# linjonathan/tropical_cyclone_risk

Measured on AMD Instinct MI355X. Metric: storm-steps/sec (100k-storm ensemble), higher is better.
Workload: dtype f64

## Files before the change

### tropical_cyclone_risk_amd/csrc/tcr_abi.hip

```cpp
#include <hip/hip_runtime.h>

#include <atomic>
#include <chrono>
#include <cmath>
#include <condition_variable>
#include <memory>
#include <mutex>
#include <thread>
#include <cstdio>
#include <cstdlib>
#include <cstring>
#include <string>
#include <vector>

#include "tcr_kernels.hip"
#include "tcr_seed.hip"
#include "tcr_compact.hip"
#include "tcr_prep.hip"
#include "tcr_thermo.hip"
#ifdef TCR_EXPERIMENTS
#include "tcr_experiments.h"
#endif

using namespace tcr;
// ... 611 lines not shown
    const bool f64 = std::is_same<R, double>::value;
    if (ctx->split_static) { K.bx = axis_of<R>(ctx->bg, true); K.by = axis_of<R>(ctx->bg, false); }
    else { K.bx = K.hx; K.by = K.hy; }
    switch (ctx->static_mode) {
    case kStatF64Split:
        K.stat = f64 ? static_cast<const void *>(ctx->d_land) : static_cast<const void *>(ctx->d_land32);
        K.bathy = f64 ? static_cast<const void *>(ctx->d_bathy) : static_cast<const void *>(ctx->d_bathy32);
        break;
    case kStatPack16: case kStatPack64: K.stat = ctx->d_nstat; K.bathy = nullptr; break;
    case kStatU8F32: K.stat = ctx->d_nstat; K.bathy = ctx->d_nbathy; break;
    default:
        K.stat = f64 ? static_cast<const void *>(ctx->d_stat) : static_cast<const void *>(ctx->d_stat32);
        K.bathy = nullptr;
        break;
    }
    eval_k_scalars<R>(ctx->prm, K);
    K.tw_same = (ctx->wg.lon == ctx->tg.lon && ctx->wg.lat == ctx->tg.lat) ? 1 : 0;
    K.hb_same = ctx->split_static ? 0 : 1;
    *all_affine = K.wx.affine && K.wy.affine && K.tx.affine && K.ty.affine && K.hx.affine && K.hy.affine &&
                  K.bx.affine && K.by.affine;
}

int widen_static(tcr_ctx *ctx, hipStream_t st)
{
    const int mode = ctx->static_mode;
    if (mode != kStatPack16 && mode != kStatU8F32 && mode != kStatPack64) return 0;
    if (ctx->capturing) return fail(ctx, "internal: static fields would be widened inside a stream capture");
    const size_t np = ctx->hg.lon.size() * ctx->hg.lat.size();
    const size_t nb = ctx->split_static ? ctx->bg.lon.size() * ctx->bg.lat.size() : np;
    if (ctx->split_static) { if (dev_alloc(ctx, &ctx->d_land, np) || dev_alloc(ctx, &ctx->d_bathy, nb)) return -1; }
    else if (dev_alloc(ctx, &ctx->d_stat, np * kStaticStride)) return -1;
    hipLaunchKernelGGL(k_static_widen, dim3((unsigned)((std::max(np, nb) + 255) / 256)), dim3(256), 0, st, mode, ctx->d_nstat, ctx->d_nbathy,
                       np, nb, ctx->d_stat, ctx->d_land, ctx->d_bathy);
    HIPCHK(ctx, hipGetLastError());
    HIPCHK(ctx, hipStreamSynchronize(st));
    HIPCHK(ctx, hipFree(ctx->d_nstat)); ctx->d_nstat = nullptr;
    if (ctx->d_nbathy) { HIPCHK(ctx, hipFree(ctx->d_nbathy)); ctx->d_nbathy = nullptr; }
    ctx->static_mode = ctx->split_static ? kStatF64Split : kStatF64;
    ctx->static_bytes = sizeof(double) * (np + nb);
    ctx->stat32_stale = true;
    ++ctx->epoch;
    return 0;
}

template <typename R>
int eval_k_ready(tcr_ctx *ctx, EvalKT<R> &K, bool *affine, hipStream_t st)
{
    host_eval_k<R>(ctx, K, affine);
    if (!*affine && (ctx->static_mode == kStatPack16 || ctx->static_mode == kStatU8F32 || ctx->static_mode == kStatPack64)) {
        if (widen_static(ctx, st)) return -1;
        if (!std::is_same<R, double>::value && ensure_f32(ctx, st)) return -1;
        host_eval_k<R>(ctx, K, affine);
    }
    return 0;
}

template <typename R>
struct TracksT {
    R *lon, *lat, *v, *m, *vmax, *envw;
    int32_t *n_valid, *status, *flags, *nfev, *n_accept, *n_reject, *pad_state;
    int32_t tc_rows_only;
};
template <typename R, typename T>
TracksT<R> tracks_of(const T *o)
{
    TracksT<R> t{};
    t.lon = o->lon; t.lat = o->lat; t.v = o->v; t.m = o->m; t.vmax = o->vmax; t.envw = o->envw;
    t.n_valid = o->n_valid; t.status = o->status; t.flags = o->flags; t.nfev = o->nfev;
    t.n_accept = o->n_accept; t.n_reject = o->n_reject; t.pad_state = o->pad_state; t.tc_rows_only = o->tc_rows_only;
    return t;
}

constexpr int kFsSegSamples = kFsMfmaWaves * kFsMfmaColTiles * 16;
enum FsPart { kFsAll = -1, kFsFirst = 0, kFsRest = 1 };
bool fourier_on_matrix_cores(const tcr_ctx *ctx)
{
    const tcr_params &P = ctx->prm;
    return TCR_FS_MFMA && ctx->fs_period > 0 && 2 * P.n_series <= 4 * kFsMfmaKSteps && P.n_steps <= kFsMfmaMaxSamples;
}

template <typename R>
int launch_fourier(tcr_ctx *ctx, int64_t n, const int64_t *n_dev, const double *phases, R *fs, hipStream_t st,
                   FsPart part = kFsAll, const double *park = nullptr, const unsigned long long *park_count = nullptr,
                   const BatchReset *reset = nullptr)
{
    BatchReset z{};
    if (reset) z = *reset;
    if (reset && !(ctx->fs_period > 0 && fourier_on_matrix_cores(ctx)))
        hipLaunchKernelGGL(k_batch_reset, dim3((unsigned)((std::max<int64_t>(z.n_flags, z.queue_words) + 255) / 256)), dim3(256), 0, st, z);
    const tcr_params &P = ctx->prm;
    if (ctx->fs_period > 0) {
        const size_t lds = sizeof(double2) * (size_t)ctx->fs_period;
        const int64_t nf = n * 4 * (int64_t)P.n_series;
        if (part != kFsRest) {
            double *p = reinterpret_cast<double *>(ctx->d_pf);
            if (grow(ctx, &p, &ctx->pf_cap, (size_t)nf * 2)) { ctx->d_pf = nullptr; return -1; }
            ctx->d_pf = reinterpret_cast<double2 *>(p);
        } else if (!ctx->d_pf) return fail(ctx, "internal: second table segment without the first");
        if (fourier_on_matrix_cores(ctx)) {
            const int64_t tiles = (n + 3) / 4;
            const int64_t *list = nullptr;
            int list_stride = 1;
            if (part == kFsRest) {
                list = reinterpret_cast<const int64_t *>(park) + 13;
                list_stride = kParkRec;
            } else {
                double *p0 = reinterpret_cast<double *>(ctx->d_pf);
                if (grow(ctx, &p0, &ctx->pf_cap, (size_t)tiles * kFsMfmaKSteps * 64)) { ctx->d_pf = nullptr; return -1; }
                ctx->d_pf = reinterpret_cast<double2 *>(p0);
                hipLaunchKernelGGL(k_phase_factors_frag, dim3((unsigned)std::min<int64_t>(tiles, 8192)), dim3(256), 0, st, P, n, n_dev, phases, p0, nullptr, nullptr, z);
            }
            double *p = reinterpret_cast<double *>(ctx->d_pf);
            const int groups = part == kFsAll ? kFsMfmaColGroups : 1;
            int64_t want = (int64_t)ctx->cu_count * kFsMfmaWgsPerCu * (4 / kFsMfmaWaves) / groups;
#ifdef TCR_EXPERIMENTS
            want = tcr_exp::fs_workgroups(want, groups);
#endif
            const unsigned wgs = (unsigned)std::min<int64_t>(tiles, std::max<int64_t>(1, want));
            if (part == kFsRest)
                hipLaunchKernelGGL((k_fourier_mfma<R, true>), dim3(wgs, groups), dim3(64 * kFsMfmaWaves), 0, st, P, n, n_dev, ctx->fs_period,
                                   ctx->d_sc_table, p, fs, 1, list, list_stride, park_count);
            else
                hipLaunchKernelGGL((k_fourier_mfma<R, false>), dim3(wgs, groups), dim3(64 * kFsMfmaWaves), 0, st, P, n, n_dev, ctx->fs_period,
                                   ctx->d_sc_table, p, fs, 0, list, list_stride, park_count);
        } else {
            hipLaunchKernelGGL(k_phase_factors, dim3((unsigned)((nf + 255) / 256)), dim3(256), 0, st, P, n, n_dev, phases, ctx->d_pf);
            hipLaunchKernelGGL(k_fourier_periodic<R>, dim3((unsigned)n), dim3(kFsThreads), lds, st, P, n, n_dev,
                               ctx->fs_period, ctx->d_sc_table, ctx->d_pf, fs);
        }
    } else {
        const int64_t total = n * (int64_t)P.n_steps;
        hipLaunchKernelGGL(k_fourier_direct<R>, dim3((unsigned)((total + 255) / 256)), dim3(256), 0, st, P, n, n_dev, phases, fs);
    }
    HIPCHK(ctx, hipGetLastError());
    return 0;
}

template <typename R>
int integrate_impl(tcr_ctx *ctx, const tcr_storms *in, const TracksT<R> out, void *stream_, uint64_t *stats = nullptr,
                   const int64_t *stats_n_dev = nullptr, int64_t n_expected = 0)
{
    HIPCHK(ctx, hipSetDevice(ctx->device));
    const int64_t n = in->n;
    if (n < 0) return fail(ctx, "tcr_integrate: negative n");
    if (n == 0) return 0;
    hipStream_t st = stream_ ? (hipStream_t)stream_ : ctx->stream;
    const tcr_params &P = ctx->prm;
    const size_t ns = (size_t)P.n_steps;
    constexpr size_t REC = (size_t)step_rec_doubles<R>();
    if (grow(ctx, &ctx->d_fs, &ctx->fs_cap, ((size_t)n * ns * 4 * sizeof(R) + 7) / 8)) return -1;
    const int max_rk = P.max_rk_steps > 0 ? P.max_rk_steps : 64;
    if (grow(ctx, &ctx->d_srec, &ctx->srec_cap, (size_t)n * max_rk * REC)) return -1;
    if (grow(ctx, &ctx->d_vrec, &ctx->vrec_cap, (size_t)n * max_rk * kVRec)) return -1;
    if (max_rk > 65535) return fail(ctx, "tcr_params.max_rk_steps must be <= 65535");
    {
        double *p = reinterpret_cast<double *>(ctx->d_sidx);
        if (grow(ctx, &p, &ctx->sidx_cap, ((size_t)n * ns * sizeof(uint16_t) + 7) / 8)) { ctx->d_sidx = nullptr; return -1; }
        ctx->d_sidx = reinterpret_cast<uint16_t *>(p);
    }
    R *fs = reinterpret_cast<R *>(ctx->d_fs);
    EvalKT<R> EK{};
    bool affine = false;
    if (eval_k_ready<R>(ctx, EK, &affine, st)) return -1;

    hipEvent_t *ev = nullptr;
    if (ctx->timing && !ctx->capturing && timing_events(ctx, &ev)) return -1;
    if (ev) HIPCHK(ctx, hipEventRecord(ev[0], st));
    const int wps = std::is_same<R, double>::value ? TCR_INT_WPS : TCR_INT_WPS_F32;
    unsigned waves = integrate_waves(ctx, (n_expected > 0 && n_expected < n) ? n_expected : n, wps);
    const int thr = park_threshold(ctx, waves, wps);
    const unsigned final_waves = park_final_waves(ctx);
    const bool segmented = kFsMfmaColGroups == 2 && thr > 0 && waves > final_waves && kMaxPasses > 1 && fourier_on_matrix_cores(ctx) &&
                           (int)P.n_steps > kFsSegSamples + 16 && ctx->tune.table_segments != 0;
    int prune_sample = -1;
    if (out.tc_rows_only && ctx->tune.prune != 0) {
        const double t2d = 2 * 86400.0, step_out = P.total_time / (double)(P.n_steps - 1);
        const int j = (int)floor(t2d / step_out);
        if (j >= 1 && j < P.n_steps - 1 && ts_host(P, j) == t2d) {
            prune_sample = j;
            double *q = reinterpret_cast<double *>(ctx->d_screen_skip);
            if (grow(ctx, &q, &ctx->screen_skip_cap, ((size_t)n + 7) / 8)) { ctx->d_screen_skip = nullptr; return -1; }
            ctx->d_screen_skip = reinterpret_cast<uint8_t *>(q);
            double *u = reinterpret_cast<double *>(ctx->d_und_list);
            if (grow(ctx, &u, &ctx->und_list_cap, ((size_t)n + 1) / 2 + 1)) { ctx->d_und_list = nullptr; return -1; }
            ctx->d_und_list = reinterpret_cast<int32_t *>(u);
            if (!ctx->d_und_count && dev_alloc(ctx, &ctx->d_und_count, (size_t)1)) return -1;
        }
    }
    {
        BatchReset z{};
        z.queue = ctx->d_queue; z.queue_words = (int)kQueueWords;
        if (prune_sample >= 0) { z.und_count = ctx->d_und_count; z.flags = out.flags; z.n_flags = n; }
        if (out.tc_rows_only) z.tc_count = reinterpret_cast<unsigned long long *>(ctx->d_tc_count);
        if (launch_fourier<R>(ctx, n, in->n_dev, in->phases, fs, st, segmented ? kFsFirst : kFsAll, nullptr, nullptr, &z)) return -1;
    }
    STAGE(TCR_STAGE_FOURIER);
    if (ev) HIPCHK(ctx, hipEventRecord(ev[1], st));
    {
        KArgsT<R> a{};
        a.P = P; a.D = dev_fields(ctx); a.K = EK; a.n = n; a.n_dev = in->n_dev;
        a.lon0 = in->lon0; a.lat0 = in->lat0; a.v0 = in->v0; a.m0 = in->m0; a.h_bl = in->h_bl;
        a.slot = in->slot; a.phases = in->phases; a.fs = fs; a.srec = ctx->d_srec; a.vrec = ctx->d_vrec; a.max_rk_steps = max_rk;
        a.n_valid = out.n_valid; a.status = out.status; a.nfev = out.nfev;
        a.n_accept = out.n_accept; a.n_reject = out.n_reject;
        a.queue = ctx->d_queue;
        a.prune_sample = prune_sample;
        a.screen_skip = prune_sample >= 0 ? ctx->d_screen_skip : nullptr;
        if (prune_sample >= 0) {
            a.und_list = ctx->d_und_list; a.und_count = ctx->d_und_count;
        }
        const size_t park_items = segmented ? (size_t)n : (size_t)waves * kWave;
        if (thr > 0 && grow(ctx, &ctx->d_park[0], &ctx->park_cap[0], park_items * kParkRec)) return -1;
        if (thr > 0 && grow(ctx, &ctx->d_park[1], &ctx->park_cap[1], park_items * kParkRec)) return -1;
        const bool probe = std::is_same<R, double>::value && ctx->d_probe;
        if (probe) { a.probe = ctx->d_probe; a.probe_cap = ctx->probe_cap; }
        bool seg_events = false;
        for (int pass = 0; pass < kMaxPasses; ++pass) {
            const bool last = thr <= 0 || waves <= final_waves || pass == kMaxPasses - 1;
            a.pass = pass;
            a.fill_pct = pass_fill_pct();
            a.threshold = last ? 0 : thr;
            a.park_in = ctx->d_park[(pass + 1) & 1];
            a.park_out = ctx->d_park[pass & 1];
            a.t_limit = (segmented && pass == 0) ? ts_host(P, kFsSegSamples - 2) : 1e300;
            launch_integrate(a, affine, probe, ctx->static_mode, waves, st);
            if (last) break;
            if (segmented && pass == 0) {
                if (ev) HIPCHK(ctx, hipEventRecord(ev[4], st));
                if (launch_fourier<R>(ctx, n, in->n_dev, in->phases, fs, st, kFsRest, ctx->d_park[0], ctx->d_queue + kMaxPasses)) return -1;
                if (ev) HIPCHK(ctx, hipEventRecord(ev[5], st));
                seg_events = true;
                continue;
            }
            waves = (unsigned)(((size_t)waves * (size_t)(thr - 1) + kWave - 1) / kWave);
        }
        if (ev && !seg_events) { HIPCHK(ctx, hipEventRecord(ev[4], st)); HIPCHK(ctx, hipEventRecord(ev[5], st)); }
    }
    STAGE(TCR_STAGE_INTEGRATE);
    if (ev) HIPCHK(ctx, hipEventRecord(ev[2], st));
    {
        EArgsT<R> a{};
        a.P = P; a.D = dev_fields(ctx); a.n = n; a.n_dev = in->n_dev; a.max_rk_steps = max_rk; a.srec = ctx->d_srec; a.vrec = ctx->d_vrec; a.fs = fs;
        a.slot = in->slot; a.n_valid = out.n_valid; a.status = out.status; a.n_accept = out.n_accept;
        a.lon = out.lon; a.lat = out.lat; a.v = out.v; a.m = out.m; a.vmax = out.vmax;
        a.envw = out.envw; a.flags = out.flags; a.pad_state = out.pad_state;
        a.K = EK;
        a.screen_skip = prune_sample >= 0 ? ctx->d_screen_skip : nullptr;
        if (prune_sample >= 0) { a.und_list = ctx->d_und_list; a.und_count = ctx->d_und_count; }
        const unsigned chunks = (unsigned)((ns + kPostThreads - 1) / kPostThreads);
        if (out.tc_rows_only) {
            if ((size_t)n > ctx->tc_idx_cap) {
                if (ctx->d_tc_idx) HIPCHK(ctx, hipFree(ctx->d_tc_idx));
                ctx->d_tc_idx = nullptr; ctx->tc_idx_cap = 0;
                if (dev_alloc(ctx, &ctx->d_tc_idx, (size_t)n)) return -1;
                ctx->tc_idx_cap = (size_t)n;
            }
            a.tc_list = ctx->d_tc_idx; a.tc_count = reinterpret_cast<unsigned long long *>(ctx->d_tc_count);
            hipLaunchKernelGGL(k_screen<R>, dim3((unsigned)((n + kScreenStorms - 1) / kScreenStorms)), dim3(kScreenThreads), 0, st, a);
            STAGE(TCR_STAGE_SCREEN);
            STAGE(TCR_STAGE_SELECT_TC);
            a.list = ctx->d_tc_idx; a.count = ctx->d_tc_count;
        }
        int64_t cap = kEmitGridCap;
        if (ctx->tune.emit_grid_cap > 0) cap = ctx->tune.emit_grid_cap;
        const unsigned gx = (out.tc_rows_only && n > 2 * cap) ? (unsigned)cap : (unsigned)n;
        hipLaunchKernelGGL(k_dense<R>, dim3(gx), dim3(kWave), 0, st, a, ctx->d_sidx);
        STAGE(TCR_STAGE_DENSE);
        const unsigned ex = gx;
        if (out.tc_rows_only) {
            if (affine) hipLaunchKernelGGL((k_emit<R, true, false>), dim3(ex, chunks), dim3(kPostThreads), 0, st, a, ctx->d_sidx);
            else hipLaunchKernelGGL((k_emit<R, false, false>), dim3(ex, chunks), dim3(kPostThreads), 0, st, a, ctx->d_sidx);
            if ((int64_t)ex < n) {
                a.item_base = ex;
                const unsigned ov = (unsigned)std::min<int64_t>(n - ex, 256);
                if (affine) hipLaunchKernelGGL((k_emit<R, true, true>), dim3(ov, chunks), dim3(kPostThreads), 0, st, a, ctx->d_sidx);
                else hipLaunchKernelGGL((k_emit<R, false, true>), dim3(ov, chunks), dim3(kPostThreads), 0, st, a, ctx->d_sidx);
                a.item_base = 0;
// ... 868 lines not shown
        if (ctx->d_tiles) HIPCHK(ctx, hipFree(ctx->d_tiles));
        ctx->d_tiles = nullptr; ctx->tiles_cap = 0;
        if (dev_alloc(ctx, &ctx->d_tiles, (size_t)tiles + 1024)) return -1;
        HIPCHK(ctx, hipMemsetAsync(ctx->d_tiles, 0, sizeof(unsigned long long) * ((size_t)tiles + 1024), st));
        ctx->tiles_cap = (size_t)tiles + 1024;
    }
    if (cell) hipLaunchKernelGGL(k_compact<true>, dim3((unsigned)tiles), dim3(kScanThreads), 0, st, n, flags, mask, max_out, idx, count, ctx->d_tiles, (int)tiles, *cell);
    else hipLaunchKernelGGL(k_compact<false>, dim3((unsigned)tiles), dim3(kScanThreads), 0, st, n, flags, mask, max_out, idx, count, ctx->d_tiles, (int)tiles, CellOrderArgs{});
    HIPCHK(ctx, hipGetLastError());
    return 0;
}
}
}

int tcr_compact_dev(tcr_ctx *ctx, int64_t n, const int32_t *flags, int32_t mask, int64_t max_out,
                    int32_t *idx, int64_t *count, void *stream_)
{
    return compact_impl(ctx, n, flags, mask, max_out, idx, count, stream_, nullptr);
}

extern "C++" {
namespace {
int cell_order_args(tcr_ctx *ctx, const tcr_seeds *cand, int32_t *idx, int64_t n, const int64_t *count, double cell_deg,
                    hipStream_t st, CellOrderArgs &a)
{
    if (!cand || !cand->lon0 || !cand->lat0 || !idx || n < 0) return fail(ctx, "tcr_cell_order_dev: bad argument");
    if (!(cell_deg >= 0.25 && cell_deg <= 90.0)) return fail(ctx, "tcr_cell_order_dev: cell_deg must be in [0.25, 90]");
    a = CellOrderArgs{};
    a.ncol = (int)ceil(360.0 / cell_deg);
    const int nrow = (int)ceil(180.0 / cell_deg) + 1;
    a.nbins = a.ncol * nrow;
    if (a.nbins > (1 << 20)) return fail(ctx, "tcr_cell_order_dev: too many cells");
    const size_t head = 3 * ((size_t)a.nbins + 1) + 8;
    const size_t words = head + 4 * (size_t)n;
    if ((words + 1) / 2 > ctx->cell_cap || ctx->cell_bins != a.nbins) {
        if (grow(ctx, &ctx->d_cell, &ctx->cell_cap, (words + 1) / 2 + 4096)) return -1;
        HIPCHK(ctx, hipMemsetAsync(ctx->d_cell, 0, sizeof(int32_t) * head, st));
        ctx->cell_bins = a.nbins;
        ctx->cell_counts_open = false;
    } else if (ctx->cell_counts_open && !ctx->capturing) {
        HIPCHK(ctx, hipMemsetAsync(ctx->d_cell, 0, sizeof(int32_t) * head, st));
        ctx->cell_counts_open = false;
    }
    int32_t *w = reinterpret_cast<int32_t *>(ctx->d_cell);
    a.hist = w; a.start = w + a.nbins + 1; a.long_cells = w + 2 * (a.nbins + 1);
    int32_t *body = w + head;
    a.idx_in = body; a.key = body + n; a.tmp = body + 2 * n; a.tmp_key = body + 3 * n;
    a.lon0 = cand->lon0; a.lat0 = cand->lat0; a.idx_out = idx; a.count = count; a.n = n;
    a.inv_cell = 1.0 / cell_deg;
    return 0;
}

int cell_order_launch(tcr_ctx *ctx, const CellOrderArgs &a, bool key_done, hipStream_t st)
{
    const int64_t n = a.n;
    const unsigned blocks = (unsigned)((n + 255) / 256);
    ctx->cell_counts_open = true;
    if (!key_done) hipLaunchKernelGGL(k_cell_key, dim3(blocks), dim3(256), 0, st, a);
    hipLaunchKernelGGL(k_cell_scan, dim3(1), dim3(kCellScanThreads), 0, st, a);
    hipLaunchKernelGGL(k_cell_scatter, dim3(blocks), dim3(256), 0, st, a);
    hipLaunchKernelGGL(k_cell_rank, dim3((unsigned)((std::max<int64_t>(n, a.nbins + 1) + 255) / 256)), dim3(256), 0, st, a);
    HIPCHK(ctx, hipGetLastError());
    ctx->cell_counts_open = false;
    return 0;
}
}
}

int tcr_cell_order_dev(tcr_ctx *ctx, const tcr_seeds *cand, int32_t *idx, int64_t n, const int64_t *count,
                       double cell_deg, void *stream_)
{
    if (!ctx) return -1;
    HIPCHK(ctx, hipSetDevice(ctx->device));
    hipStream_t st = stream_ ? (hipStream_t)stream_ : ctx->stream;
    CellOrderArgs a{};
    if (cell_order_args(ctx, cand, idx, n, count, cell_deg, st, a)) return -1;
    if (n == 0) return 0;
    return cell_order_launch(ctx, a, false, st);
}

extern "C++" {
namespace {
int gather_impl(tcr_ctx *ctx, const tcr_seeds *src, const int32_t *idx, int64_t n_out, const int64_t *count,
                const tcr_seeds *dst, uint64_t experiment_seed, int32_t year, int64_t cand0, const RoundKey *key, void *stream_)
{
    if (!ctx) return -1;
    if (!ctx->have_prm) return fail(ctx, "tcr_params_set has not been called");
    if (!src || !dst || !idx) return fail(ctx, "tcr_gather_seeds_dev: NULL argument");
    HIPCHK(ctx, hipSetDevice(ctx->device));
    if (n_out <= 0) return 0;
    hipStream_t st = stream_ ? (hipStream_t)stream_ : ctx->stream;
    GatherSeedArgs a{};
    a.src = *src; a.dst = *dst; a.idx = idx; a.n_out = n_out; a.phases_per_storm = 4 * ctx->prm.n_series;
    a.seed = experiment_seed; a.year = year; a.cand0 = cand0; a.count = count; a.key = key;
    const int64_t threads = n_out * kGatherLanes;
    hipLaunchKernelGGL(k_gather_seeds, dim3((unsigned)((threads + 255) / 256)), dim3(256), 0, st, a);
    HIPCHK(ctx, hipGetLastError());
    return 0;
}
}
}

int tcr_gather_seeds_dev(tcr_ctx *ctx, const tcr_seeds *src, const int32_t *idx, int64_t n_out,
                         const int64_t *count, const tcr_seeds *dst, uint64_t experiment_seed, int32_t year,
                         int64_t cand0, void *stream_)
{
    return gather_impl(ctx, src, idx, n_out, count, dst, experiment_seed, year, cand0, nullptr, stream_);
}

int tcr_stats_dev(tcr_ctx *ctx, int64_t n, const int64_t *n_dev, const tcr_tracks *t, uint64_t *out, int32_t n_out, void *stream_)
{
    if (!ctx) return -1;
    if (!t || !out) return fail(ctx, "tcr_stats_dev: NULL argument");
    if (n_out != 6 && n_out != 8 && n_out != TCR_N_STATS) return fail(ctx, "tcr_stats_dev: n_out must be 6, 8 or 10 (the capacity of out_dev in words)");
    HIPCHK(ctx, hipSetDevice(ctx->device));
    if (n <= 0) return 0;
    hipStream_t st = stream_ ? (hipStream_t)stream_ : ctx->stream;
    int64_t blocks = (n + 255) / 256;
    if (blocks > 512) blocks = 512;
    hipLaunchKernelGGL(k_stats, dim3((unsigned)blocks), dim3(256), 0, st, n, n_dev, t->n_valid, t->nfev, t->flags, t->status,
                       reinterpret_cast<unsigned long long *>(out), (int)n_out);
    HIPCHK(ctx, hipGetLastError());
    return 0;
}

extern "C++" {
namespace {
template <typename R, typename T>
int pack_impl(tcr_ctx *ctx, const T *src, const int32_t *idx, const int64_t *count, int64_t cap, double *packed,
              int64_t row_stride, void *stream_, const int32_t *cand_idx = nullptr, const int32_t *slot = nullptr,
              const int32_t *basin_idx = nullptr, int64_t cand0 = 0, const RoundKey *key = nullptr)
{
    if (!ctx) return -1;
    if (!ctx->have_prm) return fail(ctx, "tcr_params_set has not been called");
    if (!src || !idx || !count || !packed) return fail(ctx, "tcr_pack_tracks: NULL argument");
    HIPCHK(ctx, hipSetDevice(ctx->device));
    if (cap <= 0) return 0;
    hipStream_t st = stream_ ? (hipStream_t)stream_ : ctx->stream;
    PackArgsT<R> a{};
    a.lon = src->lon; a.lat = src->lat; a.v = src->v; a.m = src->m; a.vmax = src->vmax; a.envw = src->envw;
    a.idx = idx; a.count = count; a.cap = cap; a.ns = ctx->prm.n_steps; a.packed = packed;
    a.row_stride = row_stride > 0 ? row_stride : 9 * (int64_t)ctx->prm.n_steps;
    if (a.row_stride < 9 * (int64_t)ctx->prm.n_steps) return fail(ctx, "tcr_pack_tracks: row_stride < 9 * n_steps");
    if (slot) {
        if (!basin_idx) return fail(ctx, "tcr_pack_tracks_meta_dev: slot and basin_idx go together");
        if (a.row_stride < 9 * (int64_t)ctx->prm.n_steps + 3) return fail(ctx, "tcr_pack_tracks_meta_dev: row_stride < 9 * n_steps + 3");
        a.cand_idx = cand_idx; a.slot = slot; a.basin_idx = basin_idx; a.cand0 = cand0; a.key = key;
    }
    hipLaunchKernelGGL(k_pack_tracks<R>, dim3((unsigned)cap), dim3(256), 0, st, a);
    HIPCHK(ctx, hipGetLastError());
    return 0;
}
}
}

int tcr_pack_tracks_dev(tcr_ctx *ctx, const tcr_tracks *src, const int32_t *idx, const int64_t *count,
                        int64_t cap, double *packed, int64_t row_stride, void *stream_)
{
    return pack_impl<double>(ctx, src, idx, count, cap, packed, row_stride, stream_);
}

int tcr_pack_tracks_f32_dev(tcr_ctx *ctx, const tcr_tracks_f32 *src, const int32_t *idx, const int64_t *count,
                            int64_t cap, double *packed, int64_t row_stride, void *stream_)
{
    return pack_impl<float>(ctx, src, idx, count, cap, packed, row_stride, stream_);
}

int tcr_pack_tracks_meta_dev(tcr_ctx *ctx, const tcr_tracks *src, int32_t f32, const int32_t *idx, const int64_t *count,
                             int64_t cap, double *packed, int64_t row_stride, const int32_t *cand_idx, const int32_t *slot,
                             const int32_t *basin_idx, int64_t cand0, void *stream_)
{
    if (ctx && (!slot || !basin_idx)) return fail(ctx, "tcr_pack_tracks_meta_dev: NULL argument");
    if (f32) return pack_impl<float>(ctx, reinterpret_cast<const tcr_tracks_f32 *>(src), idx, count, cap, packed, row_stride, stream_,
                                     cand_idx, slot, basin_idx, cand0);
    return pack_impl<double>(ctx, src, idx, count, cap, packed, row_stride, stream_, cand_idx, slot, basin_idx, cand0);
}

extern "C++" {
namespace {
int seed_hist_impl(tcr_ctx *ctx, const tcr_seeds *cand, int64_t n, int64_t cand0, const RoundKey *key, const double *cutoff,
                   int64_t *out, void *stream_)
{
    if (!ctx) return -1;
    if (!cand || !cand->seed_flags || !cand->basin_idx || !cand->slot || !out) return fail(ctx, "tcr_seed_hist_dev: NULL argument");
    HIPCHK(ctx, hipSetDevice(ctx->device));
    hipStream_t st = stream_ ? (hipStream_t)stream_ : ctx->stream;
    SeedHistArgs a{};
    a.seed_flags = cand->seed_flags; a.basin_idx = cand->basin_idx; a.slot = cand->slot; a.n = n > 0 ? n : 0; a.cand0 = cand0;
    a.key = key; a.cutoff = cutoff; a.out = reinterpret_cast<unsigned long long *>(out);
    if (!ctx->d_hist_partial) {
        const size_t words = (size_t)kSeedHistBlocks * TCR_N_BASINS * 12 + 16;
        if (dev_alloc(ctx, &ctx->d_hist_partial, words)) return -1;
        HIPCHK(ctx, hipMemsetAsync(ctx->d_hist_partial, 0, sizeof(unsigned int) * words, st));
    }
    a.partial = ctx->d_hist_partial;
    const int64_t blocks = std::max<int64_t>(1, std::min<int64_t>(kSeedHistBlocks, (a.n + 1023) / 1024));
    hipLaunchKernelGGL(k_seed_hist, dim3((unsigned)blocks), dim3(256), 0, st, a);
    HIPCHK(ctx, hipGetLastError());
    return 0;
}

int enqueue_round(tcr_ctx *ctx, const tcr_round *r, uint64_t seed, int32_t year, int64_t cand0, const RoundKey *key, void *st)
{
    tcr_seeds cand = r->cand, storms = r->storms;
    cand.n = r->n_cand; storms.n = r->n_storms;
    STAGE(TCR_STAGE_START);
    if (seed_impl(ctx, seed, year, cand0, key, &cand, st)) return -1;
    STAGE(TCR_STAGE_SEED);
#ifdef TCR_EXPERIMENTS
    tcr_exp::dummy_launches((hipStream_t)st, reinterpret_cast<unsigned long long *>(ctx->d_cell));
#endif
    if (r->cell_deg > 0) {
        CellOrderArgs ca{};
        if (cell_order_args(ctx, &cand, r->cand_idx, r->n_storms, r->n_passed, r->cell_deg, (hipStream_t)st, ca)) return -1;
        const bool fused = ca.nbins > kCellLdsBins;
        if (fused) ctx->cell_counts_open = true;
        if (compact_impl(ctx, r->n_cand, cand.seed_flags, 2, r->n_storms, r->cand_idx, r->n_passed, st, fused ? &ca : nullptr)) return -1;
        STAGE(TCR_STAGE_SELECT);
        if (cell_order_launch(ctx, ca, fused, (hipStream_t)st)) return -1;
    } else {
        if (compact_impl(ctx, r->n_cand, cand.seed_flags, 2, r->n_storms, r->cand_idx, r->n_passed, st, nullptr)) return -1;
        STAGE(TCR_STAGE_SELECT);
    }
    STAGE(TCR_STAGE_ORDER);
    if (gather_impl(ctx, &cand, r->cand_idx, r->n_storms, r->n_passed, &storms, seed, year, cand0, key, st)) return -1;
    STAGE(TCR_STAGE_GATHER);
    tcr_storms in{};
    in.n = r->n_storms; in.lon0 = storms.lon0; in.lat0 = storms.lat0; in.v0 = storms.v0; in.m0 = storms.m0; in.h_bl = storms.h_bl;
    in.slot = storms.slot; in.phases = storms.phases; in.n_dev = r->exact_count ? r->n_passed : nullptr;
    if (r->f32) {
        if (ensure_f32(ctx, (hipStream_t)st)) return -1;
        if (integrate_impl<float>(ctx, &in, tracks_of<float>(reinterpret_cast<const tcr_tracks_f32 *>(&r->tracks)), st, r->stats, r->n_passed, r->n_expected)) return -1;
    } else if (integrate_impl<double>(ctx, &in, tracks_of<double>(&r->tracks), st, r->stats, r->n_passed, r->n_expected)) return -1;
    STAGE(TCR_STAGE_STATS);
    if (r->acc_idx) {
        if (!r->n_accepted) return fail(ctx, "tcr_round_dev: acc_idx without n_accepted");
        if (tcr_compact_dev(ctx, r->n_storms, r->tracks.flags, TCR_FLAG_ACCEPTED, r->n_storms, r->acc_idx, r->n_accepted, st)) return -1;
        if (r->packed && r->pack_cap > 0) {
            const bool meta = r->pack_stride >= 9 * (int64_t)ctx->prm.n_steps + 3;
            const int32_t *ci = meta ? r->cand_idx : nullptr, *sl = meta ? storms.slot : nullptr, *bi = meta ? storms.basin_idx : nullptr;
            if (r->f32 ? pack_impl<float>(ctx, reinterpret_cast<const tcr_tracks_f32 *>(&r->tracks), r->acc_idx, r->n_accepted, r->pack_cap,
                                          r->packed, r->pack_stride, st, ci, sl, bi, cand0, key)
                       : pack_impl<double>(ctx, &r->tracks, r->acc_idx, r->n_accepted, r->pack_cap, r->packed, r->pack_stride, st,
                                           ci, sl, bi, cand0, key)) return -1;
        }
    }
    if (r->seed_hist && seed_hist_impl(ctx, &cand, r->n_cand, cand0, key, nullptr, r->seed_hist, st)) return -1;
    STAGE(TCR_STAGE_PACK);
    return 0;
}

void drop_graphs(tcr_ctx *ctx)
{
    for (auto &g : ctx->graphs) { if (g.exec) (void)hipGraphExecDestroy(g.exec); if (g.graph) (void)hipGraphDestroy(g.graph); }
    ctx->graphs.clear();
}
}
}

int tcr_seed_hist_dev(tcr_ctx *ctx, const tcr_seeds *cand, int64_t cand0, const double *cutoff, int64_t *out, void *stream_)
{
    return seed_hist_impl(ctx, cand, cand ? cand->n : 0, cand0, nullptr, cutoff, out, stream_);
}

int tcr_round_dev(tcr_ctx *ctx, const tcr_round *r, uint64_t seed, int32_t year, int64_t cand0, int32_t use_graph, void *stream_)
{
    if (ready(ctx, true)) return -1;
    if (!r) return fail(ctx, "tcr_round_dev: NULL argument");
    if (r->n_cand <= 0 || r->n_storms <= 0) return fail(ctx, "tcr_round_dev: n_cand and n_storms must be positive");
    if (r->n_storms > r->n_cand) return fail(ctx, "tcr_round_dev: n_storms > n_cand");
    if (!r->cand_idx || !r->n_passed || !r->cand.seed_flags || !r->cand.lon0 || !r->storms.lon0 || !r->storms.phases ||
        !r->storms.basin_idx || !r->tracks.flags || !r->tracks.n_valid)
        return fail(ctx, "tcr_round_dev: NULL buffer");
    if (r->cell_deg != 0 && !(r->cell_deg >= 0.25 && r->cell_deg <= 90.0)) return fail(ctx, "tcr_round_dev: cell_deg must be 0 or in [0.25, 90]");
    HIPCHK(ctx, hipSetDevice(ctx->device));
    hipStream_t st = stream_ ? (hipStream_t)stream_ : ctx->stream;
    if (!use_graph || ctx->d_probe) return enqueue_round(ctx, r, seed, year, cand0, nullptr, st);

    std::vector<uint8_t> key(sizeof(tcr_round) + sizeof(uint64_t) + sizeof(void *));
    memcpy(key.data(), r, sizeof(tcr_round));
    {
        constexpr size_t pad0 = offsetof(tcr_round, tracks) + offsetof(tcr_tracks, tc_rows_only) + sizeof(int32_t);
        constexpr size_t pad1 = offsetof(tcr_round, tracks) + sizeof(tcr_tracks);
        static_assert(pad1 >= pad0 && sizeof(tcr_seeds) == 80 && sizeof(tcr_round) == 384, "tcr_round layout changed: revisit the key");
        memset(key.data() + pad0, 0, pad1 - pad0);
    }
    memcpy(key.data() + sizeof(tcr_round), &ctx->epoch, sizeof(uint64_t));
    memcpy(key.data() + sizeof(tcr_round) + sizeof(uint64_t), &st, sizeof(void *));
    tcr_ctx::RoundGraph *g = nullptr;
    for (auto &c : ctx->graphs) if (c.key == key) { g = &c; break; }
    if (!g) {
        if (!ctx->graphs.empty() && memcmp(ctx->graphs.front().key.data() + sizeof(tcr_round), &ctx->epoch, sizeof(uint64_t)) != 0)
            drop_graphs(ctx);
        if (ctx->graphs.size() >= 64) drop_graphs(ctx);
        if (enqueue_round(ctx, r, seed, year, cand0, nullptr, st)) return -1;
        memcpy(key.data() + sizeof(tcr_round), &ctx->epoch, sizeof(uint64_t));
        ctx->graphs.emplace_back();
        g = &ctx->graphs.back();
        g->key = key;
        if (hipStreamBeginCapture(st, hipStreamCaptureModeThreadLocal) != hipSuccess) { g->failed = true; (void)hipGetLastError(); return 0; }
        ctx->capturing = true;
        const int rc = enqueue_round(ctx, r, 0, 0, 0, ctx->d_round_key, st);
        ctx->capturing = false;
        hipGraph_t graph = nullptr;
        hipError_t e = hipStreamEndCapture(st, &graph);
        hipStreamCaptureStatus cs = hipStreamCaptureStatusNone;
        if (hipStreamIsCapturing(st, &cs) == hipSuccess && cs != hipStreamCaptureStatusNone) {
            hipGraph_t junk = nullptr;
            (void)hipStreamEndCapture(st, &junk);
            if (junk) (void)hipGraphDestroy(junk);
            e = hipErrorStreamCaptureInvalidated;
        }
        for (int k = 0; k < 4 && hipGetLastError() != hipSuccess; ++k) {}
        if (rc || e != hipSuccess || !graph) {
            if (graph) (void)hipGraphDestroy(graph);
            ctx->err.clear();
// ... 94 lines not shown
```

### tropical_cyclone_risk_amd/csrc/tcr_compact.hip

```cpp
#include "tcr_device.h"
#include "tcr_seed.hip"

namespace tcr {

constexpr int kScanThreads = 256;
constexpr int kScanItems = 8;
constexpr int kScanTile = kScanThreads * kScanItems;

struct CellOrderArgs {
    const double *lon0, *lat0;
    int32_t *idx_in;
    int32_t *idx_out;
    const int64_t *count;
    int64_t n;
    double inv_cell;
    int ncol, nbins;
    int32_t *key;
    int32_t *hist;
    int32_t *start;
    int32_t *tmp, *tmp_key;
    int32_t *long_cells;
};

constexpr int kCellLong = 96;
// ... 18 lines not shown
    __hip_atomic_store(p, v, __ATOMIC_RELEASE, __HIP_MEMORY_SCOPE_AGENT);
}

template <bool KEY>
__global__ __launch_bounds__(kScanThreads) void k_compact(int64_t n, const int32_t *__restrict__ flags, int32_t mask,
                                                          int64_t max_out, int32_t *__restrict__ idx, int64_t *__restrict__ total,
                                                          unsigned long long *__restrict__ state, int n_tiles, CellOrderArgs cell)
{
    __shared__ int s[kScanThreads];
    __shared__ int s_tile;
    __shared__ unsigned s_gen;
    __shared__ long long s_prefix[kScanThreads / 64];
    if (threadIdx.x == 0) {
        s_tile = (int)__hip_atomic_fetch_add(state, 1ull, __ATOMIC_RELAXED, __HIP_MEMORY_SCOPE_AGENT);
        s_gen = (unsigned)ld_agent(state + 1) + 1u;
    }
    __syncthreads();
    const int tile = s_tile;
    const unsigned gen = s_gen;
    const int64_t base = (int64_t)tile * kScanTile + (int64_t)threadIdx.x * kScanItems;
    int c = 0;
    bool sel[kScanItems];
#pragma unroll
    for (int k = 0; k < kScanItems; ++k) {
        const int64_t i = base + k;
        sel[k] = i < n && (flags[i] & mask);
        c += sel[k];
    }
    s[threadIdx.x] = c;
    __syncthreads();
    for (int off = 1; off < kScanThreads; off <<= 1) {
        const int t = threadIdx.x >= off ? s[threadIdx.x - off] : 0;
        __syncthreads();
        s[threadIdx.x] += t;
        __syncthreads();
    }
    const int tile_total = s[kScanThreads - 1];
    if (threadIdx.x == 0) st_agent(state + 2 + tile, ((unsigned long long)gen << 32) | (unsigned)tile_total);
    long long before = 0;
    for (int p = threadIdx.x; p < tile; p += kScanThreads) {
        unsigned long long w = ld_agent(state + 2 + p);
        while ((unsigned)(w >> 32) != gen) { __builtin_amdgcn_s_sleep(1); w = ld_agent(state + 2 + p); }
        before += (long long)(unsigned)w;
    }
    for (int off = 32; off > 0; off >>= 1) before += __shfl_down(before, off);
    if ((threadIdx.x & 63) == 0) s_prefix[threadIdx.x >> 6] = before;
    __syncthreads();
    long long prefix = 0;
#pragma unroll
    for (int w = 0; w < kScanThreads / 64; ++w) prefix += s_prefix[w];
    if (tile == n_tiles - 1 && threadIdx.x == 0) {
        *total = prefix + tile_total;
        st_agent(state, 0ull);
        st_agent(state + 1, (unsigned long long)gen);
    }
    int64_t rank = prefix + s[threadIdx.x] - c;
#pragma unroll
    for (int k = 0; k < kScanItems; ++k)
        if (sel[k]) {
            if (rank < max_out) {
                const int32_t c = (int32_t)(base + k);
                idx[rank] = c;
                if (KEY) {
                    cell.idx_in[rank] = c;
                    const int kk = cell_of(cell, cell.lon0[c], cell.lat0[c]);
                    cell.key[rank] = kk;
                    atomicAdd(cell.hist + kk, 1);
                }
            }
            ++rank;
        }
}

struct GatherSeedArgs {
    tcr_seeds src, dst;
    const int32_t *idx;
    int64_t n_out;
    int phases_per_storm;
    uint64_t seed;
    int32_t year;
    int64_t cand0;
    const int64_t *count;
    const RoundKey *key;
};

constexpr int kGatherLanes = 16;

__global__ __launch_bounds__(256) void k_gather_seeds(GatherSeedArgs a)
{
    const int64_t gid = (int64_t)blockIdx.x * blockDim.x + threadIdx.x;
    const int64_t row = gid / kGatherLanes;
    const int lane = (int)(gid % kGatherLanes);
    if (row >= a.n_out || (a.count && row >= *a.count)) return;
    const int32_t j = a.idx[row];
    if (lane == kGatherLanes - 1) {
        a.dst.lon0[row] = a.src.lon0[j]; a.dst.lat0[row] = a.src.lat0[j];
        a.dst.v0[row] = a.src.v0[j]; a.dst.m0[row] = a.src.m0[j]; a.dst.h_bl[row] = a.src.h_bl[j];
        a.dst.slot[row] = a.src.slot[j];
        if (a.dst.basin_idx) a.dst.basin_idx[row] = a.src.basin_idx[j];
        if (a.dst.seed_flags) a.dst.seed_flags[row] = a.src.seed_flags[j];
    }
    double *dp = a.dst.phases + (size_t)row * a.phases_per_storm;
    if (a.src.phases) {
        const double *sp = a.src.phases + (size_t)j * a.phases_per_storm;
        for (int k = lane; k < a.phases_per_storm; k += kGatherLanes) dp[k] = sp[k];
    } else {
        const uint64_t seed = a.key ? a.key->seed : a.seed;
        const int32_t year = a.key ? a.key->year : a.year;
        const int64_t cand0 = a.key ? a.key->cand0 : a.cand0;
        for (int p = lane; 2 * p < a.phases_per_storm; p += kGatherLanes) {
            double p0, p1;
            uniform2_raw(seed, year, cand0 + j, 2u, (uint32_t)p, p0, p1);
            dp[2 * p] = p0;
            if (2 * p + 1 < a.phases_per_storm) dp[2 * p + 1] = p1;
        }
    }
}

__device__ __forceinline__ int64_t cell_n(const CellOrderArgs &a) { return (a.count && *a.count < a.n) ? *a.count : a.n; }

constexpr int kCellLdsBins = 2048;

__global__ __launch_bounds__(256) void k_cell_key(CellOrderArgs a)
{
    __shared__ int h[kCellLdsBins];
    const bool local = a.nbins <= kCellLdsBins;
    if (local) {
        for (int b = threadIdx.x; b < a.nbins; b += 256) h[b] = 0;
        __syncthreads();
    }
    const int64_t i = (int64_t)blockIdx.x * 256 + threadIdx.x;
    if (i < cell_n(a)) {
        const int32_t c = a.idx_out[i];
        a.idx_in[i] = c;
        const int k = cell_of(a, a.lon0[c], a.lat0[c]);
        a.key[i] = k;
        if (local) atomicAdd(&h[k], 1); else atomicAdd(a.hist + k, 1);
    }
    if (local) {
        __syncthreads();
        for (int b = threadIdx.x; b < a.nbins; b += 256) if (h[b]) atomicAdd(a.hist + b, h[b]);
    }
}

constexpr int kCellScanThreads = 256;
constexpr int kCellScanRun = 64;
constexpr int kCellScanWin = kCellScanThreads * kCellScanRun;
constexpr size_t kCellScanLds = sizeof(int) * (kCellScanWin + 2 * kCellScanThreads + 1);
static_assert(kCellScanLds <= 160 * 1024, "k_cell_scan's LDS window exceeds a gfx950 CU's 160 KB");
__device__ __forceinline__ int cell_lds(int i) { return i + i / kCellScanRun; }
__global__ __launch_bounds__(kCellScanThreads) void k_cell_scan(CellOrderArgs a)
{
    __shared__ int v[kCellScanWin + kCellScanThreads];
    __shared__ int s[kCellScanThreads];
    __shared__ int n_long;
    if (threadIdx.x == 0) n_long = 0;
    int carry = 0;
    for (int base = 0; base < a.nbins; base += kCellScanWin) {
        for (int i0 = threadIdx.x; i0 < kCellScanWin; i0 += 16 * kCellScanThreads) {
            int t[16];
#pragma unroll
            for (int u = 0; u < 16; ++u) { const int i = i0 + u * kCellScanThreads; t[u] = (i < kCellScanWin && base + i < a.nbins) ? a.hist[base + i] : 0; }
#pragma unroll
            for (int u = 0; u < 16; ++u) { const int i = i0 + u * kCellScanThreads; if (i < kCellScanWin) v[cell_lds(i)] = t[u]; }
        }
        __syncthreads();
        int sum = 0;
        const int row = threadIdx.x * (kCellScanRun + 1);
#pragma unroll 8
        for (int j = 0; j < kCellScanRun; ++j) sum += v[row + j];
        s[threadIdx.x] = sum;
        __syncthreads();
        for (int off = 1; off < kCellScanThreads; off <<= 1) {
            const int t = threadIdx.x >= off ? s[threadIdx.x - off] : 0;
            __syncthreads();
            s[threadIdx.x] += t;
            __syncthreads();
        }
        int run = carry + s[threadIdx.x] - sum;
#pragma unroll 8
        for (int j = 0; j < kCellScanRun; ++j) {
            const int c = v[row + j];
            if (c > kCellLong) a.long_cells[1 + atomicAdd(&n_long, 1)] = base + threadIdx.x * kCellScanRun + j;
            v[row + j] = run; run += c;
        }
        const int total = s[kCellScanThreads - 1];
        __syncthreads();
        for (int i = threadIdx.x; i < kCellScanWin; i += kCellScanThreads)
            if (base + i < a.nbins) { const int o = v[cell_lds(i)]; a.hist[base + i] = o; a.start[base + i] = o; }
        carry += total;
        __syncthreads();
    }
    if (threadIdx.x == 0) { a.hist[a.nbins] = carry; a.start[a.nbins] = carry; a.long_cells[0] = n_long; }
}

__global__ __launch_bounds__(256) void k_cell_scatter(CellOrderArgs a)
{
// ... 214 lines not shown
```

Baseline: 10.57 billion.

## Fuse phase-factor fragment generation into the seed gather kernel

The seed gather kernel now also computes the weighted sin/cos phase factors for the matrix-core Fourier table. It stages them in shared memory per 4-row tile and writes the MFMA fragment layout directly, so the separate k_phase_factors_frag launch is skipped. The batch reset also moves into this kernel, and the gather call moves inside integrate_impl. This removes one kernel launch and a re-read of the phases, at the cost of extra shared memory, block barriers and heavier per-thread work in the gather. It also moves the timing event that marks the start of the Fourier stage.

```diff
diff --git a/tropical_cyclone_risk_amd/csrc/tcr_abi.hip b/tropical_cyclone_risk_amd/csrc/tcr_abi.hip
--- a/tropical_cyclone_risk_amd/csrc/tcr_abi.hip
+++ b/tropical_cyclone_risk_amd/csrc/tcr_abi.hip
@@ -717,10 +717,11 @@
 template <typename R>
 int launch_fourier(tcr_ctx *ctx, int64_t n, const int64_t *n_dev, const double *phases, R *fs, hipStream_t st,
                    FsPart part = kFsAll, const double *park = nullptr, const unsigned long long *park_count = nullptr,
-                   const BatchReset *reset = nullptr)
+                   const BatchReset *reset = nullptr, bool frag_done = false)
 {
     BatchReset z{};
     if (reset) z = *reset;
+    if (frag_done && !fourier_on_matrix_cores(ctx)) return fail(ctx, "internal: fragments without the matrix-core table");
     if (reset && !(ctx->fs_period > 0 && fourier_on_matrix_cores(ctx)))
         hipLaunchKernelGGL(k_batch_reset, dim3((unsigned)((std::max<int64_t>(z.n_flags, z.queue_words) + 255) / 256)), dim3(256), 0, st, z);
     const tcr_params &P = ctx->prm;
@@ -743,7 +744,8 @@
                 double *p0 = reinterpret_cast<double *>(ctx->d_pf);
                 if (grow(ctx, &p0, &ctx->pf_cap, (size_t)tiles * kFsMfmaKSteps * 64)) { ctx->d_pf = nullptr; return -1; }
                 ctx->d_pf = reinterpret_cast<double2 *>(p0);
-                hipLaunchKernelGGL(k_phase_factors_frag, dim3((unsigned)std::min<int64_t>(tiles, 8192)), dim3(256), 0, st, P, n, n_dev, phases, p0, nullptr, nullptr, z);
+                if (!frag_done)
+                    hipLaunchKernelGGL(k_phase_factors_frag, dim3((unsigned)std::min<int64_t>(tiles, 8192)), dim3(256), 0, st, P, n, n_dev, phases, p0, nullptr, nullptr, z);
             }
             double *p = reinterpret_cast<double *>(ctx->d_pf);
             const int groups = part == kFsAll ? kFsMfmaColGroups : 1;
@@ -771,9 +773,27 @@
     return 0;
 }
 
+struct RoundGather {
+    const tcr_seeds *src, *dst;
+    const int32_t *idx;
+    const int64_t *count;
+    uint64_t seed;
+    int32_t year;
+    int64_t cand0;
+    const RoundKey *key;
+};
+struct GatherFrag {
+    double *frag;
+    const int64_t *n_dev;
+    BatchReset reset;
+};
+int gather_impl(tcr_ctx *ctx, const tcr_seeds *src, const int32_t *idx, int64_t n_out, const int64_t *count,
+                const tcr_seeds *dst, uint64_t experiment_seed, int32_t year, int64_t cand0, const RoundKey *key, void *stream_,
+                const GatherFrag *gf = nullptr);
+
 template <typename R>
 int integrate_impl(tcr_ctx *ctx, const tcr_storms *in, const TracksT<R> out, void *stream_, uint64_t *stats = nullptr,
-                   const int64_t *stats_n_dev = nullptr, int64_t n_expected = 0)
+                   const int64_t *stats_n_dev = nullptr, int64_t n_expected = 0, const RoundGather *rg = nullptr)
 {
     HIPCHK(ctx, hipSetDevice(ctx->device));
     const int64_t n = in->n;
@@ -800,7 +820,6 @@
 
     hipEvent_t *ev = nullptr;
     if (ctx->timing && !ctx->capturing && timing_events(ctx, &ev)) return -1;
-    if (ev) HIPCHK(ctx, hipEventRecord(ev[0], st));
     const int wps = std::is_same<R, double>::value ? TCR_INT_WPS : TCR_INT_WPS_F32;
     unsigned waves = integrate_waves(ctx, (n_expected > 0 && n_expected < n) ? n_expected : n, wps);
     const int thr = park_threshold(ctx, waves, wps);
@@ -827,7 +846,21 @@
         z.queue = ctx->d_queue; z.queue_words = (int)kQueueWords;
         if (prune_sample >= 0) { z.und_count = ctx->d_und_count; z.flags = out.flags; z.n_flags = n; }
         if (out.tc_rows_only) z.tc_count = reinterpret_cast<unsigned long long *>(ctx->d_tc_count);
-        if (launch_fourier<R>(ctx, n, in->n_dev, in->phases, fs, st, segmented ? kFsFirst : kFsAll, nullptr, nullptr, &z)) return -1;
+        const bool frag_done = rg && fourier_on_matrix_cores(ctx);
+        if (rg) {
+            GatherFrag gf{};
+            if (frag_done) {
+                double *p = reinterpret_cast<double *>(ctx->d_pf);
+                const size_t need = std::max((size_t)n * 4 * (size_t)P.n_series * 2, (size_t)((n + 3) / 4) * kFsMfmaKSteps * 64);
+                if (grow(ctx, &p, &ctx->pf_cap, need)) { ctx->d_pf = nullptr; return -1; }
+                ctx->d_pf = reinterpret_cast<double2 *>(p);
+                gf.frag = p; gf.n_dev = in->n_dev; gf.reset = z;
+            }
+            if (gather_impl(ctx, rg->src, rg->idx, n, rg->count, rg->dst, rg->seed, rg->year, rg->cand0, rg->key, st, frag_done ? &gf : nullptr)) return -1;
+            STAGE(TCR_STAGE_GATHER);
+        }
+        if (ev) HIPCHK(ctx, hipEventRecord(ev[0], st));
+        if (launch_fourier<R>(ctx, n, in->n_dev, in->phases, fs, st, segmented ? kFsFirst : kFsAll, nullptr, nullptr, &z, frag_done)) return -1;
     }
     STAGE(TCR_STAGE_FOURIER);
     if (ev) HIPCHK(ctx, hipEventRecord(ev[1], st));
@@ -1862,7 +1895,8 @@
 extern "C++" {
 namespace {
 int gather_impl(tcr_ctx *ctx, const tcr_seeds *src, const int32_t *idx, int64_t n_out, const int64_t *count,
-                const tcr_seeds *dst, uint64_t experiment_seed, int32_t year, int64_t cand0, const RoundKey *key, void *stream_)
+                const tcr_seeds *dst, uint64_t experiment_seed, int32_t year, int64_t cand0, const RoundKey *key, void *stream_,
+                const GatherFrag *gf)
 {
     if (!ctx) return -1;
     if (!ctx->have_prm) return fail(ctx, "tcr_params_set has not been called");
@@ -1874,7 +1908,13 @@
     a.src = *src; a.dst = *dst; a.idx = idx; a.n_out = n_out; a.phases_per_storm = 4 * ctx->prm.n_series;
     a.seed = experiment_seed; a.year = year; a.cand0 = cand0; a.count = count; a.key = key;
     const int64_t threads = n_out * kGatherLanes;
-    hipLaunchKernelGGL(k_gather_seeds, dim3((unsigned)((threads + 255) / 256)), dim3(256), 0, st, a);
+    if (gf) {
+        const int N = ctx->prm.n_series;
+        if (N > 16 || !gf->frag) return fail(ctx, "internal: seed gather asked for fragments the matrix-core table cannot take");
+        a.frag = gf->frag; a.n_dev = gf->n_dev; a.n_series = N; a.reset = gf->reset;
+        for (int h = 0; h < N; ++h) a.fs_wgt[h] = ctx->prm.fs_wgt[h];
+        hipLaunchKernelGGL(k_gather_seeds<true>, dim3((unsigned)((threads + 255) / 256)), dim3(256), 0, st, a);
+    } else hipLaunchKernelGGL(k_gather_seeds<false>, dim3((unsigned)((threads + 255) / 256)), dim3(256), 0, st, a);
     HIPCHK(ctx, hipGetLastError());
     return 0;
 }
@@ -2003,15 +2043,15 @@
         STAGE(TCR_STAGE_SELECT);
     }
     STAGE(TCR_STAGE_ORDER);
-    if (gather_impl(ctx, &cand, r->cand_idx, r->n_storms, r->n_passed, &storms, seed, year, cand0, key, st)) return -1;
-    STAGE(TCR_STAGE_GATHER);
+    const RoundGather rg{&cand, &storms, r->cand_idx, r->n_passed, seed, year, cand0, key};
+    if (r->n_storms <= 0) STAGE(TCR_STAGE_GATHER);
     tcr_storms in{};
     in.n = r->n_storms; in.lon0 = storms.lon0; in.lat0 = storms.lat0; in.v0 = storms.v0; in.m0 = storms.m0; in.h_bl = storms.h_bl;
     in.slot = storms.slot; in.phases = storms.phases; in.n_dev = r->exact_count ? r->n_passed : nullptr;
     if (r->f32) {
         if (ensure_f32(ctx, (hipStream_t)st)) return -1;
-        if (integrate_impl<float>(ctx, &in, tracks_of<float>(reinterpret_cast<const tcr_tracks_f32 *>(&r->tracks)), st, r->stats, r->n_passed, r->n_expected)) return -1;
-    } else if (integrate_impl<double>(ctx, &in, tracks_of<double>(&r->tracks), st, r->stats, r->n_passed, r->n_expected)) return -1;
+        if (integrate_impl<float>(ctx, &in, tracks_of<float>(reinterpret_cast<const tcr_tracks_f32 *>(&r->tracks)), st, r->stats, r->n_passed, r->n_expected, &rg)) return -1;
+    } else if (integrate_impl<double>(ctx, &in, tracks_of<double>(&r->tracks), st, r->stats, r->n_passed, r->n_expected, &rg)) return -1;
     STAGE(TCR_STAGE_STATS);
     if (r->acc_idx) {
         if (!r->n_accepted) return fail(ctx, "tcr_round_dev: acc_idx without n_accepted");
diff --git a/tropical_cyclone_risk_amd/csrc/tcr_compact.hip b/tropical_cyclone_risk_amd/csrc/tcr_compact.hip
--- a/tropical_cyclone_risk_amd/csrc/tcr_compact.hip
+++ b/tropical_cyclone_risk_amd/csrc/tcr_compact.hip
@@ -124,37 +124,86 @@
     int64_t cand0;
     const int64_t *count;
     const RoundKey *key;
+    double *frag;
+    const int64_t *n_dev;
+    int n_series;
+    double fs_wgt[16];
+    BatchReset reset;
 };
 
 constexpr int kGatherLanes = 16;
-
+constexpr int kGatherStage = 64 + 8;
+static_assert(kGatherLanes * 4 == 64, "a wave of k_gather_seeds is one row tile of the fragments");
+
+template <bool FRAG>
 __global__ __launch_bounds__(256) void k_gather_seeds(GatherSeedArgs a)
 {
+    __shared__ double stage[FRAG ? 4 : 1][FRAG ? kFsMfmaKSteps * kGatherStage : 1];
     const int64_t gid = (int64_t)blockIdx.x * blockDim.x + threadIdx.x;
     const int64_t row = gid / kGatherLanes;
     const int lane = (int)(gid % kGatherLanes);
-    if (row >= a.n_out || (a.count && row >= *a.count)) return;
-    const int32_t j = a.idx[row];
-    if (lane == kGatherLanes - 1) {
-        a.dst.lon0[row] = a.src.lon0[j]; a.dst.lat0[row] = a.src.lat0[j];
-        a.dst.v0[row] = a.src.v0[j]; a.dst.m0[row] = a.src.m0[j]; a.dst.h_bl[row] = a.src.h_bl[j];
-        a.dst.slot[row] = a.src.slot[j];
-        if (a.dst.basin_idx) a.dst.basin_idx[row] = a.src.basin_idx[j];
-        if (a.dst.seed_flags) a.dst.seed_flags[row] = a.src.seed_flags[j];
-    }
+    double *const w = stage[FRAG ? threadIdx.x >> 6 : 0];
+    if (FRAG) {
+        batch_reset(a.reset, gid, (int64_t)gridDim.x * blockDim.x);
+#pragma unroll
+        for (int u = 0; u < kFsMfmaKSteps; ++u) w[u * kGatherStage + (threadIdx.x & 63)] = 0.0;
+        __syncthreads();
+    }
+    const bool valid = row < a.n_out && !(a.count && row >= *a.count);
+    if (!FRAG && !valid) return;
+    const int N = a.n_series;
+    auto factors = [&](int k, double x) {
+        const int s = k / N, h = k - s * N;
+        const double wgt = a.fs_wgt[h];
+        const double sb = wgt * sinpi(2.0 * x), cb = wgt * cospi(2.0 * x);
+        const int kk = 2 * h;
+        double *o = w + (kk >> 2) * kGatherStage + s * 4 + (int)(row & 3);
+        o[(kk & 3) * 16] = cb;
+        o[((kk & 3) + 1) * 16] = sb;
+    };
+    const int64_t ne = FRAG ? n_eff(a.n_out, a.n_dev) : 0;
     double *dp = a.dst.phases + (size_t)row * a.phases_per_storm;
-    if (a.src.phases) {
-        const double *sp = a.src.phases + (size_t)j * a.phases_per_storm;
-        for (int k = lane; k < a.phases_per_storm; k += kGatherLanes) dp[k] = sp[k];
-    } else {
-        const uint64_t seed = a.key ? a.key->seed : a.seed;
-        const int32_t year = a.key ? a.key->year : a.year;
-        const int64_t cand0 = a.key ? a.key->cand0 : a.cand0;
-        for (int p = lane; 2 * p < a.phases_per_storm; p += kGatherLanes) {
-            double p0, p1;
-            uniform2_raw(seed, year, cand0 + j, 2u, (uint32_t)p, p0, p1);
-            dp[2 * p] = p0;
-            if (2 * p + 1 < a.phases_per_storm) dp[2 * p + 1] = p1;
+    if (valid) {
+        const int32_t j = a.idx[row];
+        if (lane == kGatherLanes - 1) {
+            a.dst.lon0[row] = a.src.lon0[j]; a.dst.lat0[row] = a.src.lat0[j];
+            a.dst.v0[row] = a.src.v0[j]; a.dst.m0[row] = a.src.m0[j]; a.dst.h_bl[row] = a.src.h_bl[j];
+            a.dst.slot[row] = a.src.slot[j];
+            if (a.dst.basin_idx) a.dst.basin_idx[row] = a.src.basin_idx[j];
+            if (a.dst.seed_flags) a.dst.seed_flags[row] = a.src.seed_flags[j];
+        }
+        if (a.src.phases) {
+            const double *sp = a.src.phases + (size_t)j * a.phases_per_storm;
+            for (int k = lane; k < a.phases_per_storm; k += kGatherLanes) {
+                const double x = sp[k];
+                dp[k] = x;
+                if (FRAG && row < ne) factors(k, x);
+            }
+        } else {
+            const uint64_t seed = a.key ? a.key->seed : a.seed;
+            const int32_t year = a.key ? a.key->year : a.year;
+            const int64_t cand0 = a.key ? a.key->cand0 : a.cand0;
+            for (int p = lane; 2 * p < a.phases_per_storm; p += kGatherLanes) {
+                double p0, p1;
+                uniform2_raw(seed, year, cand0 + j, 2u, (uint32_t)p, p0, p1);
+                dp[2 * p] = p0;
+                if (FRAG && row < ne) factors(2 * p, p0);
+                if (2 * p + 1 < a.phases_per_storm) {
+                    dp[2 * p + 1] = p1;
+                    if (FRAG && row < ne) factors(2 * p + 1, p1);
+                }
+            }
+        }
+    } else if (FRAG && row < ne) {
+        for (int k = lane; k < a.phases_per_storm; k += kGatherLanes) factors(k, dp[k]);
+    }
+    if (FRAG) {
+        __syncthreads();
+        const int64_t tile = gid >> 6;
+        if (tile < (ne + 3) / 4) {
+            double *o = a.frag + tile * (kFsMfmaKSteps * 64) + (threadIdx.x & 63);
+#pragma unroll
+            for (int u = 0; u < kFsMfmaKSteps; ++u) o[u * 64] = w[u * kGatherStage + (threadIdx.x & 63)];
         }
     }
 }
```

After: 10.61 billion, median of 6. Within noise of the previous version (+0.4%).
